# HazyResearch/flash-fft-conv

Measured on NVIDIA H100. Metric: fftconv_fwd_convs_per_sec, higher is better.
Workload: dtype bf16

## Files before the change

### flash-fft-conv_b200/csrc/fwd3_r128.cuh

```cuda
#pragma once
#include "r128_common.cuh"
#include <type_traits>

namespace bffc {
namespace r128 {

constexpr int kPipes3 = 2;
constexpr int kThreads3 = kPipes3 * kPipeThreads;
constexpr int kSmemData3 = kPipes3 * 2 * kSlotBytes;
constexpr int kSmemBars3 = 128;
constexpr int kSmemTwSt3 = 128 * 8;
constexpr int kSmemRows3 = kPipeThreads * 4;

enum Phase {
  kPhTmaWait, kPhPass0, kPhStage1, kPhBarStage1, kPhPass1, kPhStage2, kPhKfWait, kPhPass3, kPhStage3, kPhPass5,
  kPhBarPass5, kPhStoreY, kPhPublishY, kPhStage4, kPhBarStage4, kPhGateWait, kPhPass6, kPhPublishOut, kPhStoreOut,
  kPhases
};
#ifdef BFFC_PHASE_CLOCK
__device__ unsigned long long* g_phase_buf;
__device__ int g_phase_one_pipe;
constexpr int kSmemClock3 = kPipes3 * kPhases * 8;
struct PhaseClock {
  uint32_t row;
  long long t;
  DEVINL void init(uint32_t s) {
    row = s;
    for (int i = 0; i < kPhases; ++i) st_shared_u64(row + 8u * i, 0ull);
    t = clock64();
  }
  DEVINL void mark(int ph) {
    const long long now = clock64();
    st_shared_u64(row + 8u * ph, ld_shared_u64(row + 8u * ph) + uint64_t(now - t));
    t = clock64();
  }
  DEVINL void flush(int pipe, int units) {
    if (g_phase_buf == nullptr) return;
    unsigned long long* g = g_phase_buf + pipe * (kPhases + 1);
    for (int i = 0; i < kPhases; ++i) atomicAdd(g + i, ld_shared_u64(row + 8u * i));
    atomicAdd(g + kPhases, (unsigned long long)units);
  }
};
#else
constexpr int kSmemClock3 = 0;
#endif

constexpr int kSmemKb3 = kThreads3 * 4;
constexpr int kSmemTotal3 =
    kSmemData3 + kSmemF + kSmemG + kSmemBars3 + kSmemTwSt3 + kSmemRows3 + kSmemClock3 + kSmemKb3 + 1024;
static_assert(kSmemTotal3 <= 227 * 1024, "shared memory per block");

struct GateMaps { CUtensorMap pre, post, post2, y2, xg; };

struct ShortRow {
  bool valid, lvalid, rvalid;
  template <class P>
  DEVINL ShortRow(const P& p, int g, int row) {
    const int r = row & 127, rblk = p.seg_bytes >> 7, sg = r / rblk, ris = r - sg * rblk, used = p.L >> 6;
    valid = (g * p.nseg + sg) * 2 + (row >> 7) < p.B && ris < used;
    lvalid = ris > 0;
    rvalid = ris + 1 < used;
  }
};

template <int kFmt, class Sync>
DEVINL void short_slot(uint32_t sA, uint32_t sB, const Taps& ta, const Taps& tb, bool fa, bool fb, int row,
                       const ShortRow& g, Sync&& sync) {
  using NT = Num<kFmt>;
  const uint4 z = make_uint4(0u, 0u, 0u, 0u);
  auto at = [&](uint32_t s, int r, int c) { return s + uint32_t(r) * 128u + (uint32_t(c ^ (r & 7)) << 4); };
  uint4 la = z, ra = z, lb = z, rb = z;
  if (g.valid && g.lvalid) {
    la = ld_shared_v4(at(sA, row - 1, 7));
    if (sB) lb = ld_shared_v4(at(sB, row - 1, 7));
  }
  if (g.valid && g.rvalid) {
    ra = ld_shared_v4(at(sA, row + 1, 0));
    if (sB) rb = ld_shared_v4(at(sB, row + 1, 0));
  }
  sync();
  if (!g.valid) return;
  uint4 pa = la, ca = ld_shared_v4(at(sA, row, 0)), pb = lb, cb = sB ? ld_shared_v4(at(sB, row, 0)) : z;
#pragma unroll 1
  for (int c = 0; c < 8; ++c) {
    const uint4 na = c < 7 ? ld_shared_v4(at(sA, row, c + 1)) : ra;
    const uint4 nb = !sB ? z : c < 7 ? ld_shared_v4(at(sB, row, c + 1)) : rb;
    uint4 o = fa ? short8<kFmt>(pa, ca, na, ta) : ca;
    if (sB) {
      const uint4 q = fb ? short8<kFmt>(pb, cb, nb, tb) : cb;
      o = make_uint4(NT::hmul2(o.x, q.x), NT::hmul2(o.y, q.y), NT::hmul2(o.z, q.z), NT::hmul2(o.w, q.w));
    }
    st_shared_v4(at(sA, row, c), o.x, o.y, o.z, o.w);
    pa = ca; ca = na; pb = cb; cb = nb;
  }
}

template <bool kPlanes, bool kGated, int kFmt, bool kShort = false>
__global__ void __launch_bounds__(kThreads3, 1)
fwd3_kernel(const __grid_constant__ CUtensorMap tm_u, const __grid_constant__ CUtensorMap tm_y,
            const __grid_constant__ CUtensorMap tm_g, const __grid_constant__ GateMaps gm,
            const std::conditional_t<kShort, FwdShortParams, FwdParams> p) {
  static_assert(!(kPlanes && kGated), "composite sizes apply their gates in the outer stages");
  static_assert(!kShort || kGated, "the short filter runs in the gated pipeline");
  constexpr bool kBlocks = !kShort;
  constexpr bool kKfSlot = !kGated && !kPlanes;
  using NT = Num<kFmt>;
  extern __shared__ uint8_t smem_raw[];
  const uint32_t sbase = (smem_u32(smem_raw) + 1023u) & ~1023u;
  uint8_t* gen_base = smem_raw + (sbase - smem_u32(smem_raw));
  const uint32_t s_f = sbase + kSmemData3;
  const uint32_t s_g = s_f + kSmemF;
  const uint32_t s_bars = s_g + kSmemG;
  const uint32_t s_twb = s_g + 3 * kGTileBytes;
  const uint32_t s_tws = s_bars + kSmemBars3;
  const uint32_t s_rows = s_tws + kSmemTwSt3;
  auto s_kb = [&]() { return s_rows + kSmemRows3 + kSmemClock3 + 4u * threadIdx.x; };

  const int tid = threadIdx.x;
  const int pipe = __shfl_sync(0xffffffffu, tid >> 8, 0);
  const int hf = __shfl_sync(0xffffffffu, (tid >> 7) & 1, 0);
  const int ptid = tid & 255;
  const bool leader = ptid == 0;
  auto frag = [&]() { return FragPos::unpack(tid, ld_shared_u32(s_rows + 4u * uint32_t(ptid))); };

  const uint32_t bar_tma0 = s_bars + pipe * 16;
  const uint32_t bar_g = s_bars + 32;
  const uint32_t bar_kf = s_bars + 40 + pipe * 8;

  if (tid == 0) {
    tma_prefetch_desc(&tm_u);
    tma_prefetch_desc(&tm_y);
    if (kPlanes) tma_prefetch_desc(&tm_g);
    if (kGated) {
      tma_prefetch_desc(&gm.pre); tma_prefetch_desc(&gm.post); tma_prefetch_desc(&gm.post2); tma_prefetch_desc(&gm.y2);
      tma_prefetch_desc(&gm.xg);
    }
    mbar_init(bar_g, 1);
  }
  if (leader) {
    mbar_init(bar_tma0, 1);
    mbar_init(bar_tma0 + 8, 1);
    if (kKfSlot) mbar_init(bar_kf, 1);
  }
  fence_barrier_init();
  __syncthreads();

  const bool has_pre = kGated && p.pregate != nullptr, has_post = kGated && p.postgate != nullptr;
  const bool has_post2 = kGated && p.y2 != nullptr;
  const bool emit_xg = has_pre && p.xg_out != nullptr;
  const uint32_t bar_gate = bar_tma0 + 8;
  uint32_t gate_phase = 0;

  const int gp = blockIdx.x * kPipes3 + pipe;
  const int GP = gridDim.x * kPipes3;
#ifdef BFFC_PHASE_CLOCK
  const bool one_pipe = g_phase_one_pipe != 0;
#else
  constexpr bool one_pipe = false;
#endif
  const int u_begin = one_pipe ? (pipe ? 0 : int((long long)p.units * blockIdx.x / gridDim.x))
                               : int((long long)p.units * gp / GP);
  const int u_end = one_pipe ? (pipe ? 0 : int((long long)p.units * (blockIdx.x + 1) / gridDim.x))
                             : int((long long)p.units * (gp + 1) / GP);
  const uint32_t s_slot0 = sbase + pipe * 2 * kSlotBytes;

  auto seq_index = [&](int unit) {
    const int h = unit / p.pairs, pr = unit - h * p.pairs;
    return pr * p.H + h;
  };
  auto issue_load = [&](int unit, int slot) {
    const uint32_t bar = bar_tma0 + 8 * slot;
    const uint32_t dst = s_slot0 + slot * kSlotBytes;
    if (kGated) {
      const int uh = unit / p.pairs, ug = unit - uh * p.pairs;
      mbar_expect_tx(bar_tma0, has_pre ? 2 * kSlotBytes : kSlotBytes);
      load_tile<false, kBlocks>(s_slot0, &tm_u, bar_tma0, uh, ug, 0, p, p.win);
      load_tile<false, kBlocks>(s_slot0 + kTileBytes, &tm_u, bar_tma0, uh, ug, 1, p, p.win);
      if (has_pre) {
        load_tile<false, kBlocks>(s_slot0 + kSlotBytes, &gm.pre, bar_tma0, uh, ug, 0, p, p.win);
        load_tile<false, kBlocks>(s_slot0 + kSlotBytes + kTileBytes, &gm.pre, bar_tma0, uh, ug, 1, p, p.win);
      }
      return;
    }
    mbar_expect_tx(bar, kSlotBytes);
    if (kPlanes) {
      tma_load_3d(dst, &tm_u, bar, 0, 0, seq_index(unit));
      tma_load_3d(dst + kTileBytes, &tm_g, bar, 0, 0, seq_index(unit));
    } else {
      const int uh = unit / p.pairs, ug = unit - uh * p.pairs;
      load_tile<false, kBlocks>(dst, &tm_u, bar, uh, ug, 0, p, p.win);
      load_tile<false, kBlocks>(dst + kTileBytes, &tm_u, bar, uh, ug, 1, p, p.win);
    }
  };
  auto kf_row = [&](int h) { return reinterpret_cast<const uint8_t*>(p.kf) + size_t(h) * kSlotBytes; };
  auto kf_block = [&](int h) {
    if (kPlanes && p.kf_gs == 1) return h;
    const uint32_t c = kPlanes ? uint32_t(p.kf_h0 + (h >> p.kf_rshift)) : uint32_t(h);
    const int g = int(__umulhi(c << 1, p.kf_gs_mul) >> p.kf_gs_shift);
    return kPlanes ? (g << p.kf_rshift) | (h & ((1 << p.kf_rshift) - 1)) : g;
  };
  if (!kKfSlot && leader && u_begin < u_end) issue_load(u_begin, 0);
  if (tid == 0) {
    mbar_expect_tx(bar_g, 3 * kGTileBytes);
    for (int c = 0; c < 3 * kGTileBytes; c += 8192)
      bulk_load(s_g + c, reinterpret_cast<const uint8_t*>(p.gtiles) + c, 8192, bar_g);
  }
  load_dft128(gen_base + kSmemData3, p.dft, tid, kThreads3);
  if (pipe == 0) {
    const FragPos fp(tid, kPlanes ? 128 : p.seg_bytes >> 7);
    st_shared_u32(s_rows + 4u * uint32_t(ptid), fp.packed());
    const float tw_inv = 1.0f / float(p.tw_n);
#pragma unroll
    for (int rr = 0; rr < 2; ++rr) {
      RowTw t;
      t.init(fp.row[rr] & p.tw_mask, fp.q, tw_inv);
      t.store(s_twb, s_tws, fp.row[rr], fp.q);
    }
  }
  auto row_tw = [&](RowTw (&tw)[2]) {
    const FragPos fp = frag();
    tw[0].load(s_twb, s_tws, fp.row[0], fp.q);
    tw[1].load(s_twb, s_tws, fp.row[1], fp.q);
  };
  if constexpr (kKfSlot) {
    grid_dep_wait();
    grid_dep_launch();
    if (leader && u_begin < u_end) {
      issue_load(u_begin, 0);
      const int g0 = kf_block(u_begin / p.pairs);
      bulk_prefetch_l2(kf_row(g0), kSlotBytes);
      if ((g0 + 1) * p.kf_gs * p.pairs < u_end) bulk_prefetch_l2(kf_row(g0 + 1), kSlotBytes);
    }
  }
  fence_proxy_async_smem();
  __syncthreads();
  mbar_wait(bar_g, 0);

  const uint32_t bar_id = 1 + pipe;
  auto pipe_sync = [&]() { named_bar_sync(bar_id, kPipeThreads); };
  auto publish_smem = [&]() { fence_proxy_async_smem(); pipe_sync(); };

  auto store_tiles = [&](const CUtensorMap* my, uint32_t sT, int unit) {
    const int uh = unit / p.pairs, ug = unit - uh * p.pairs;
    for (int w = 0; w < 2; ++w) {
      if constexpr (!kBlocks) {
        for (int sg = 0; sg < p.nseg; ++sg) {
          const int i = (ug * p.nseg + sg) * 2 + w;
          if (i < p.B) {
            const ItemPos<kBlocks> it(p, i, 0);
            tma_store_4d(my, sT + w * kTileBytes + sg * p.seg_bytes + (kBlocks ? p.win * 128 : 0), 0, it.row, uh,
                         it.b);
          }
        }
      } else {
        const ItemPos<kBlocks> it(p, ug * p.nseg * 2 + w, 0);
        for (int sg = 0; sg < p.nseg; ++sg)
          if ((ug * p.nseg + sg) * 2 + w < p.B)
            tma_store_4d(my, sT + w * kTileBytes + sg * p.seg_bytes + p.win * 128, 0, it.row, uh, it.b + 2 * sg);
      }
    }
    tma_store_commit();
  };

  Acc d;
  d.zero();
  uint32_t are[4][4], aim[4][4];
#ifdef BFFC_PHASE_CLOCK
  PhaseClock clk;
  if (leader) clk.init(s_rows + kSmemRows3 + pipe * kPhases * 8);
  auto mark = [&](int ph) { if (leader) clk.mark(ph); };
#else
  auto mark = [](int) {};
#endif

  const int kf_units = p.kf_gs * p.pairs;
  int kf_g = kKfSlot ? kf_block(u_begin / p.pairs) : 0;
  int kf_next = (kf_g + 1) * kf_units;
  for (int unit = u_begin, n = 0; unit < u_end; ++unit, ++n) {
    const int slot = kGated ? 0 : (n & 1);
    const uint32_t sX = s_slot0 + slot * kSlotBytes;
    const uint32_t sGate = s_slot0 + kSlotBytes;
    const int h = unit / p.pairs;
    if constexpr (kGated) st_shared_u32(s_kb(), uint32_t(kf_block(h)));

    mbar_wait(bar_tma0 + 8 * slot, kGated ? (n & 1) : ((n >> 1) & 1));
    mark(kPhTmaWait);
    if (kGated) {
      if constexpr (kShort) {
        const ShortParams& sf = p.sf;
        if (has_pre || sf.u.w) {
          const Taps ta = sf.u.w ? load_taps(sf.u, sf, h) : Taps{};
          const Taps tb = has_pre && sf.pre.w ? load_taps(sf.pre, sf, h) : Taps{};
          short_slot<kFmt>(sX, has_pre ? sGate : 0u, ta, tb, sf.u.w != nullptr, sf.pre.w != nullptr, ptid,
                           ShortRow(p, unit - h * p.pairs, ptid), pipe_sync);
          publish_smem();
        }
      } else if (has_pre) {
#pragma unroll 4
        for (int i = 0; i < kSlotBytes / 16 / kPipeThreads; ++i) {
          const uint32_t off = uint32_t(i * kPipeThreads + ptid) * 16u;
          const uint4 a = ld_shared_v4(sX + off), g = ld_shared_v4(sGate + off);
          st_shared_v4(sX + off, NT::hmul2(a.x, g.x), NT::hmul2(a.y, g.y), NT::hmul2(a.z, g.z), NT::hmul2(a.w, g.w));
        }
        publish_smem();
      }
      if (leader) {
        if (emit_xg) store_tiles(&gm.xg, sX, unit);
        if (has_post) {
          const int ug = unit - h * p.pairs;
          mbar_expect_tx(bar_gate, kSlotBytes);
          load_tile<false, kBlocks>(sGate, &gm.post, bar_gate, h, ug, 0, p, p.win);
          load_tile<false, kBlocks>(sGate + kTileBytes, &gm.post, bar_gate, h, ug, 1, p, p.win);
        }
      }
    }
    mark(kPhPass0);

    f128_stage<kFmt>(d, s_f, hf, sX, p.kmask);
    f128_wait<false>(d, frag());
    mark(kPhStage1);
    if constexpr (kKfSlot) pipe_sync();
    if (leader) {
      if (kGated) {
        if (emit_xg) tma_store_wait_read0();
      } else {
        if constexpr (kKfSlot) {
          mbar_expect_tx(bar_kf, kSlotBytes);
          if (unit == kf_next) { ++kf_g; kf_next += kf_units; }
          bulk_load(sX, kf_row(kf_g), kSlotBytes, bar_kf);
          if (unit == kf_next - kf_units && kf_next < u_end) bulk_prefetch_l2(kf_row(kf_g + 1), kSlotBytes);
        }
        if (unit + 1 < u_end) {
          tma_store_wait_read0();
          issue_load(unit + 1, slot ^ 1);
        }
      }
    }
    mark(kPhBarStage1);

    {
      RowTw tw[2];
      row_tw(tw);
      twiddle_frag<false>(d, tw, p.tw_scale);
    }
    frag_to_a<kFmt>(d, are, aim);
    mark(kPhPass1);
    r64_stage<kFmt>(d, are, aim, s_g, s_g + 2 * kGTileBytes, s_g + kGTileBytes, s_g);
    wgmma_wait_regs(d);
    mark(kPhStage2);

    if constexpr (kKfSlot) mbar_wait(bar_kf, n & 1);
    mark(kPhKfWait);
    {
      const FragPos fp = frag();
      const uint2* kfp = reinterpret_cast<const uint2*>(p.kf) + size_t(kGated ? int(ld_shared_u32(s_kb())) : kf_block(h)) * 16 * 128 * 2 +
                         (fp.q & 1);
      const uint32_t kfs = sX + 8u * uint32_t(fp.q & 1);
      const f32x2 kfs2 = pk2(p.kf_scale, p.kf_scale);
#pragma unroll
      for (int rr = 0; rr < 2; ++rr) {
        const int k1 = fp.row[rr];
        uint2 kv[8];
#pragma unroll
        for (int i = 0; i < 8; ++i) {
          if constexpr (kKfSlot) kv[i] = ld_shared_v2(kfs + uint32_t((2 * i + (fp.q >> 1)) * 128 + k1) * 16u);
          else kv[i] = __ldg(kfp + ((2 * i + (fp.q >> 1)) * 128 + k1) * 2);
        }
#pragma unroll
        for (int i = 0; i < 8; ++i) {
          f32x2 kr2 = NT::unpack(kv[i].x), ki2 = NT::unpack(kv[i].y ^ p.kf_conj_mask);
          if (kFmt == 0) { kr2 = mul2(kr2, kfs2); ki2 = mul2(ki2, kfs2); }
          const int e = 4 * i + 2 * rr;
          f32x2 vr, vi;
          cmul2(pk2(d.r[e], d.r[e + 1]), pk2(d.i[e], d.i[e + 1]), kr2, ki2, vr, vi);
          upk2(vr, d.r[e], d.r[e + 1]);
          upk2(vi, d.i[e], d.i[e + 1]);
        }
      }
    }
    frag_to_a<kFmt>(d, are, aim);
    mark(kPhPass3);
    r64_stage<kFmt>(d, are, aim, s_g, s_g + kGTileBytes, s_g + 2 * kGTileBytes, s_g);
    wgmma_wait_regs(d);
    mark(kPhStage3);

    {
      RowTw tw[2];
      row_tw(tw);
      twiddle_frag<true>(d, tw, p.tw_scale);
    }
    mark(kPhPass5);
    pipe_sync();
    mark(kPhBarPass5);
    frag_store_tile<kFmt>(sX, frag(), d);
    mark(kPhStoreY);
    publish_smem();
    mark(kPhPublishY);
    f128_stage<kFmt>(d, s_f, hf, sX, 0xff);
    wgmma_wait_regs(d);
    mark(kPhStage4);
    pipe_sync();
    mark(kPhBarStage4);

    auto pass6 = [&](bool gate) {
      const FragPos fp = frag();
#pragma unroll
      for (int i = 0; i < 8; ++i) {
        float o[2][2][2];
#pragma unroll
        for (int e = 0; e < 2; ++e) {
          float pr = d.r[4 * i + e], pi = d.i[4 * i + e], qr = d.r[4 * i + 2 + e], qi = d.i[4 * i + 2 + e];
          pair_butterfly<true>(fp.mix, pr, pi, qr, qi);
          o[0][0][e] = pr; o[0][1][e] = pi; o[1][0][e] = qr; o[1][1][e] = qi;
        }
#pragma unroll
        for (int rr = 0; rr < 2; ++rr) {
          const uint32_t off = frag_off(fp.row[rr], i, fp.q);
          uint32_t vr = NT::pack(o[rr][0][0], o[rr][0][1]), vi = NT::pack(o[rr][1][0], o[rr][1][1]);
          if (kGated && gate) {
            vr = NT::hmul2(vr, ld_shared_u32(sGate + off));
            vi = NT::hmul2(vi, ld_shared_u32(sGate + kTileBytes + off));
          }
          st_shared_u32(sX + off, vr);
          st_shared_u32(sX + kTileBytes + off, vi);
        }
      }
    };
    auto store_out = [&](const CUtensorMap* my) {
      if (kPlanes) {
        tma_store_3d(my, sX, 0, 0, seq_index(unit));
        tma_store_3d(&tm_g, sX + kTileBytes, 0, 0, seq_index(unit));
        tma_store_commit();
      } else {
        store_tiles(my, sX, unit);
      }
    };
    if (has_post) { mbar_wait(bar_gate, gate_phase); gate_phase ^= 1; }
    if constexpr (kShort) {
      if (has_post && p.sf.post.w) {
        const Taps tq = load_taps(p.sf.post, p.sf, h);
        short_slot<kFmt>(sGate, 0u, tq, tq, true, false, ptid, ShortRow(p, unit - h * p.pairs, ptid), pipe_sync);
        pipe_sync();
      }
    }
    mark(kPhGateWait);
    pass6(has_post);
    mark(kPhPass6);
    publish_smem();
    mark(kPhPublishOut);
    if (leader) {
      store_out(&tm_y);
      if (has_post2) {
        const int ug = unit - h * p.pairs;
        mbar_expect_tx(bar_gate, kSlotBytes);
        load_tile<false, kBlocks>(sGate, &gm.post2, bar_gate, h, ug, 0, p, p.win);
        load_tile<false, kBlocks>(sGate + kTileBytes, &gm.post2, bar_gate, h, ug, 1, p, p.win);
        tma_store_wait_read0();
      }
    }
    if (has_post2) {
      pipe_sync();
      mbar_wait(bar_gate, gate_phase); gate_phase ^= 1;
      if constexpr (kShort) {
        if (p.sf.post2.w) {
          const Taps tq = load_taps(p.sf.post2, p.sf, h);
          short_slot<kFmt>(sGate, 0u, tq, tq, true, false, ptid, ShortRow(p, unit - h * p.pairs, ptid), pipe_sync);
          pipe_sync();
        }
      }
      pass6(true);
      publish_smem();
      if (leader) store_out(&gm.y2);
    }
    if (kGated && leader && unit + 1 < u_end) {
      tma_store_wait_read0();
      issue_load(unit + 1, 0);
    }
    mark(kPhStoreOut);
  }

  if (leader) tma_store_wait_all0();
#ifdef BFFC_PHASE_CLOCK
  if (leader) clk.flush(pipe, u_end - u_begin);
#endif
}

}
}
```

Baseline: 48.06 million.

## Move next-unit TMA load to a dedicated loader thread with incremental unit indexing

In the kernel-in-slot path, the next unit's input load moves to a separate loader thread (ptid 128) and is issued after pass 5 instead of after stage 1. The leader now waits for outstanding store reads during the r64 stage. A UnitPos struct tracks head, group and block indices incrementally, replacing per-unit divisions in the load and store address math. The point is to spread TMA issue across threads and overlap the prefetch with compute, at the cost of more complex slot-reuse ordering that now depends on the store wait happening before the later load.

```diff
diff --git a/flash-fft-conv_b200/csrc/fwd3_r128.cuh b/flash-fft-conv_b200/csrc/fwd3_r128.cuh
--- a/flash-fft-conv_b200/csrc/fwd3_r128.cuh
+++ b/flash-fft-conv_b200/csrc/fwd3_r128.cuh
@@ -60,6 +60,28 @@
     valid = (g * p.nseg + sg) * 2 + (row >> 7) < p.B && ris < used;
     lvalid = ris > 0;
     rvalid = ris + 1 < used;
+  }
+};
+
+struct UnitPos {
+  int h, g, b, j;
+  struct Item { int row, b; };
+  template <class P>
+  DEVINL UnitPos(const P& p, int unit) : h(unit / p.pairs) {
+    g = unit - h * p.pairs;
+    const int i = g * p.nseg * 2;
+    b = i / p.nblk;
+    j = i - b * p.nblk;
+  }
+  template <class P>
+  DEVINL void next(const P& p) {
+    if (++g == p.pairs) { ++h; g = b = j = 0; }
+    else if (p.nblk == 1) b += 2 * p.nseg;
+    else if ((j += 2) >= p.nblk) { j -= p.nblk; ++b; }
+  }
+  template <class P>
+  DEVINL Item item(const P& p, int w) const {
+    return w && j + 1 == p.nblk ? Item{0, b + 1} : Item{(j + w) * p.srows, b};
   }
 };
 
@@ -121,6 +143,7 @@
   const int hf = __shfl_sync(0xffffffffu, (tid >> 7) & 1, 0);
   const int ptid = tid & 255;
   const bool leader = ptid == 0;
+  const bool loader = kKfSlot ? ptid == 128 : leader;
   auto frag = [&]() { return FragPos::unpack(tid, ld_shared_u32(s_rows + 4u * uint32_t(ptid))); };
 
   const uint32_t bar_tma0 = s_bars + pipe * 16;
@@ -183,13 +206,17 @@
       return;
     }
     mbar_expect_tx(bar, kSlotBytes);
-    if (kPlanes) {
-      tma_load_3d(dst, &tm_u, bar, 0, 0, seq_index(unit));
-      tma_load_3d(dst + kTileBytes, &tm_g, bar, 0, 0, seq_index(unit));
-    } else {
-      const int uh = unit / p.pairs, ug = unit - uh * p.pairs;
-      load_tile<false, kBlocks>(dst, &tm_u, bar, uh, ug, 0, p, p.win);
-      load_tile<false, kBlocks>(dst + kTileBytes, &tm_u, bar, uh, ug, 1, p, p.win);
+    tma_load_3d(dst, &tm_u, bar, 0, 0, seq_index(unit));
+    tma_load_3d(dst + kTileBytes, &tm_g, bar, 0, 0, seq_index(unit));
+  };
+  auto load_unit = [&](const UnitPos& at, int slot) {
+    const uint32_t bar = bar_tma0 + 8 * slot;
+    const uint32_t dst = s_slot0 + slot * kSlotBytes;
+    mbar_expect_tx(bar, kSlotBytes);
+    for (int w = 0; w < 2; ++w) {
+      const UnitPos::Item it = at.item(p, w);
+      for (int s = 0; s < p.nseg; ++s)
+        tma_load_4d(dst + w * kTileBytes + s * p.seg_bytes, &tm_u, bar, 0, it.row - p.win, at.h, it.b + 2 * s);
     }
   };
   auto kf_row = [&](int h) { return reinterpret_cast<const uint8_t*>(p.kf) + size_t(h) * kSlotBytes; };
@@ -222,12 +249,13 @@
     tw[0].load(s_twb, s_tws, fp.row[0], fp.q);
     tw[1].load(s_twb, s_tws, fp.row[1], fp.q);
   };
+  UnitPos at(p, u_begin);
   if constexpr (kKfSlot) {
     grid_dep_wait();
     grid_dep_launch();
-    if (leader && u_begin < u_end) {
-      issue_load(u_begin, 0);
-      const int g0 = kf_block(u_begin / p.pairs);
+    if (loader && u_begin < u_end) {
+      load_unit(at, 0);
+      const int g0 = kf_block(at.h);
       bulk_prefetch_l2(kf_row(g0), kSlotBytes);
       if ((g0 + 1) * p.kf_gs * p.pairs < u_end) bulk_prefetch_l2(kf_row(g0 + 1), kSlotBytes);
     }
@@ -261,6 +289,15 @@
     }
     tma_store_commit();
   };
+  auto store_unit = [&](const CUtensorMap* my, const UnitPos& at, uint32_t sT) {
+    for (int w = 0; w < 2; ++w) {
+      const UnitPos::Item it = at.item(p, w);
+      for (int sg = 0; sg < p.nseg; ++sg)
+        if ((at.g * p.nseg + sg) * 2 + w < p.B)
+          tma_store_4d(my, sT + w * kTileBytes + sg * p.seg_bytes + p.win * 128, 0, it.row, at.h, it.b + 2 * sg);
+    }
+    tma_store_commit();
+  };
 
   Acc d;
   d.zero();
@@ -274,7 +311,7 @@
 #endif
 
   const int kf_units = p.kf_gs * p.pairs;
-  int kf_g = kKfSlot ? kf_block(u_begin / p.pairs) : 0;
+  int kf_g = kKfSlot ? kf_block(at.h) : 0;
   int kf_next = (kf_g + 1) * kf_units;
   for (int unit = u_begin, n = 0; unit < u_end; ++unit, ++n) {
     const int slot = kGated ? 0 : (n & 1);
@@ -319,21 +356,20 @@
     f128_stage<kFmt>(d, s_f, hf, sX, p.kmask);
     f128_wait<false>(d, frag());
     mark(kPhStage1);
-    if constexpr (kKfSlot) pipe_sync();
-    if (leader) {
+    if constexpr (kKfSlot) {
+      pipe_sync();
+      if (unit == kf_next) { ++kf_g; kf_next += kf_units; }
+      if (loader) {
+        mbar_expect_tx(bar_kf, kSlotBytes);
+        bulk_load(sX, kf_row(kf_g), kSlotBytes, bar_kf);
+        if (unit == kf_next - kf_units && kf_next < u_end) bulk_prefetch_l2(kf_row(kf_g + 1), kSlotBytes);
+      }
+    } else if (leader) {
       if (kGated) {
         if (emit_xg) tma_store_wait_read0();
-      } else {
-        if constexpr (kKfSlot) {
-          mbar_expect_tx(bar_kf, kSlotBytes);
-          if (unit == kf_next) { ++kf_g; kf_next += kf_units; }
-          bulk_load(sX, kf_row(kf_g), kSlotBytes, bar_kf);
-          if (unit == kf_next - kf_units && kf_next < u_end) bulk_prefetch_l2(kf_row(kf_g + 1), kSlotBytes);
-        }
-        if (unit + 1 < u_end) {
-          tma_store_wait_read0();
-          issue_load(unit + 1, slot ^ 1);
-        }
+      } else if (unit + 1 < u_end) {
+        tma_store_wait_read0();
+        issue_load(unit + 1, slot ^ 1);
       }
     }
     mark(kPhBarStage1);
@@ -381,6 +417,7 @@
     frag_to_a<kFmt>(d, are, aim);
     mark(kPhPass3);
     r64_stage<kFmt>(d, are, aim, s_g, s_g + kGTileBytes, s_g + 2 * kGTileBytes, s_g);
+    if (kKfSlot && leader) tma_store_wait_read0();
     wgmma_wait_regs(d);
     mark(kPhStage3);
 
@@ -391,6 +428,11 @@
     }
     mark(kPhPass5);
     pipe_sync();
+    if (kKfSlot && loader && unit + 1 < u_end) {
+      UnitPos nx = at;
+      nx.next(p);
+      load_unit(nx, slot ^ 1);
+    }
     mark(kPhBarPass5);
     frag_store_tile<kFmt>(sX, frag(), d);
     mark(kPhStoreY);
@@ -431,6 +473,8 @@
         tma_store_3d(my, sX, 0, 0, seq_index(unit));
         tma_store_3d(&tm_g, sX + kTileBytes, 0, 0, seq_index(unit));
         tma_store_commit();
+      } else if (kKfSlot) {
+        store_unit(my, at, sX);
       } else {
         store_tiles(my, sX, unit);
       }
@@ -477,6 +521,7 @@
       issue_load(unit + 1, 0);
     }
     mark(kPhStoreOut);
+    if constexpr (kKfSlot) at.next(p);
   }
 
   if (leader) tma_store_wait_all0();
```

Measured after the change: 49.15 million, median of 6. 2.3% higher.
